# codelaboratoryltd/bng

Measured on NVIDIA H100. Metric: Mpps, higher is better.
Workload: dtype u8/u32/u64 integer

## Files before the change

### bng_b200/csrc/common.cuh

```cuda
#pragma once

#include <cuda_runtime.h>
#include <stdint.h>

typedef unsigned long long u64;
typedef uint32_t u32;
typedef uint16_t u16;
typedef uint8_t u8;

enum {
    ST_AS = 0,
    ST_AS_ALLOWED = 0, ST_AS_DROPPED, ST_AS_LOGGED, ST_AS_V4_VIOL, ST_AS_V6_VIOL, ST_AS_UNKNOWN_MAC,
    ST_QOS = 6,
    ST_QOS_PASS_PKTS = 6, ST_QOS_DROP_PKTS, ST_QOS_PASS_BYTES, ST_QOS_DROP_BYTES,
    ST_NAT = 10,
    ST_NAT_SNAT = 10, ST_NAT_DNAT, ST_NAT_HAIRPIN, ST_NAT_DROPPED, ST_NAT_PASSED, ST_NAT_CREATED,
    ST_NAT_EXPIRED, ST_NAT_EXHAUST, ST_NAT_EIM_HIT, ST_NAT_EIM_MISS, ST_NAT_ALG, ST_NAT_CT_LOOKUPS, ST_NAT_CT_HITS,
    ST_DHCP = 23,
    ST_DHCP_TOTAL = 23, ST_DHCP_HIT, ST_DHCP_MISS, ST_DHCP_ERROR, ST_DHCP_EXPIRED, ST_DHCP_O82_PRESENT,
    ST_DHCP_O82_ABSENT, ST_DHCP_BCAST, ST_DHCP_UCAST, ST_DHCP_VLAN,
    ST_LRU_OVERFLOW = 33,
    ST_EV_LOST_SPOOF = 34,
    ST_EV_LOST_NATLOG = 35,
    ST_TABLE_FULL = 36,
    ST_NAT_COOP = 37,
    ST_NAT_SEQ = 38,
    ST_LRU_EVICT = 39,
    ST_COUNT = 40,
};

#define K_EMPTY 0xFFFFFFFFFFFFFFFFull
#define K_TOMB 0xFFFFFFFFFFFFFFFEull
#define K_BUSY 0xFFFFFFFFFFFFFFFDull

struct Tbl {
    u8 *slots;
    u32 *count;
    u32 mask;
    u32 home_mask;
    u32 slot_bytes;
    u32 voff;
    u32 max_entries;
    u32 key_size;
    u32 value_size;
    u32 vlayout;
    u32 lru;
};
#define LRU_NONE 0u
#define LRU_TS 1u
#define LRU_ANY 2u
#define LRU_WINDOW 16u

#define VL_SESSION 1u
#define VL_QOS 2u
#define QOS_RATE_COPY 8u
enum {
    SES_NAT_IP = 16,
    SES_NAT_PORT = 20,
    SES_EPOCH = 22,
    SES_OUT_LO = 24,
    SES_LAST_SEEN = 32,
    SES_ORIG_IP = 40,
    SES_STATE = 44,
    SES_ORIG_PORT = 48,
    SES_IN_LO = 56,
    SES_OUT_HI = 64,
    SES_IN_HI = 72,
    SES_CREATED = 80,
    SES_DEST_IP = 88,
    SES_DEST_PORT = 92,
    SES_PAD_A = 96,
    SES_PAD_B = 100,
};
__host__ __device__ __forceinline__ u32 ses_abi_to_slot(u32 a) {
    if (a < 4) return SES_NAT_IP + a;
    if (a < 6) return SES_NAT_PORT + (a - 4);
    if (a < 8) return SES_ORIG_PORT + (a - 6);
    if (a < 12) return SES_ORIG_IP + (a - 8);
    if (a < 16) return SES_DEST_IP + (a - 12);
    if (a < 20) return SES_DEST_PORT + (a - 16);
    if (a < 24) return SES_PAD_A + (a - 20);
    if (a < 32) return SES_LAST_SEEN + (a - 24);
    if (a < 40) return SES_CREATED + (a - 32);
    if (a < 44) return SES_OUT_LO + (a - 40);
    if (a < 48) return SES_OUT_HI + (a - 44);
    if (a < 52) return SES_IN_LO + (a - 48);
    if (a < 56) return SES_IN_HI + (a - 52);
    if (a < 60) return SES_OUT_LO + 4 + (a - 56);
    if (a < 64) return SES_OUT_HI + 4 + (a - 60);
    if (a < 68) return SES_IN_LO + 4 + (a - 64);
    if (a < 72) return SES_IN_HI + 4 + (a - 68);
    if (a < 76) return SES_STATE + (a - 72);
    return SES_PAD_B + (a - 76);
}
__host__ __device__ __forceinline__ u32 ses_hi_of(u32 lo_off) { return lo_off == SES_OUT_LO ? (u32)SES_OUT_HI : (u32)SES_IN_HI; }
#ifdef __CUDACC__
__device__ __forceinline__ void ses_touch(u8 *ses, u64 now, u32 seen, u32 epoch, bool stamped = false) {
    if (stamped) {
        atomicMax((unsigned long long *)(ses + SES_LAST_SEEN), (unsigned long long)now);
    } else if (seen != epoch) {
        *(u64 *)(ses + SES_LAST_SEEN) = now;
        *(u16 *)(ses + SES_EPOCH) = (u16)epoch;
    }
}
static __device__ __noinline__ void ses_count_carry(u8 *ses, u32 lo_off, u32 c, u32 w) {
    u64 add = w ? (1ull << 32) : 0;
    if (c) {
        add += 1;
        u64 old = atomicAdd((unsigned long long *)(ses + lo_off), 0xFFFFFFFF00000000ull);
        if ((old >> 32) == 0) add -= 1ull << 32;
    }
    if (add) atomicAdd((unsigned long long *)(ses + ses_hi_of(lo_off)), add);
}
__device__ __forceinline__ void ses_count(u8 *ses, u32 lo_off, u32 len) {
    const u64 old = atomicAdd((unsigned long long *)(ses + lo_off), 1ull | ((u64)len << 32));
    const u32 c = (u32)old == 0xFFFFFFFFu;
    const u32 w = (u32)(((old >> 32) + len + c) >> 32);
    if (c | w) ses_count_carry(ses, lo_off, c, w);
}
#endif

#define DIR_NONE 0xFFFFFFFFu
#define DIR_QOS_UNLIMITED 0x80000000u
#define DIR_SLOT_MASK 0x7FFFFFFFu

struct LpmTbl {
    u32 *ents;
    u32 *count;
    u32 max_entries;
};

struct EvRing {
    u8 *buf;
    u32 *count;
    u32 cap;
    u32 rec_bytes;
    u32 lost_stat;
    u32 pad;
};

struct DevCtx {
    Tbl bindings;
    Tbl qos_eg;
    Tbl qos_in;
    Tbl sub_nat;
    Tbl sessions;
    Tbl reverse;
    Tbl eim;
    Tbl hairpin;
    Tbl alg;
    Tbl sub_pools;
    Tbl vlan_pools;
    Tbl cid_subs;
    Tbl ip_pools;
    Tbl cid_map;
    Tbl subdir;
    LpmTbl ranges_v4;
    LpmTbl priv_ranges;
    u8 *as_config;
    u8 *nat_config;
    u8 *server_config;
    u8 *nat_pool;
    u64 *stats;
    EvRing spoof_ev;
    EvRing natlog_ev;
    const struct SmallTabs *small;
    u32 batch_seq;
    u32 epoch;
};

#define HP_SLOTS 2048
#define HP_EMPTY 0xFFFFFFFFu
struct __align__(16) SmallTabs {
    u32 as_cfg;
    u32 nat_flags;
    u32 alg_n;
    u32 hp_n;
    u32 alg_key[64];
    u8 alg_type[64];
    u32 hp_hash[HP_SLOTS];
};
static_assert(sizeof(SmallTabs) % 16 == 0, "bulk copies move multiples of 16 bytes");

__host__ __device__ __forceinline__ u32 hp_index(u32 ip) { return (ip * 0x9E3779B1u) >> 21; }

struct DevBatch {
    u8 *pkts;
    const u32 *off16;
    u32 *len;
    u8 *verdict;
    u32 *priority;
    u32 n;
    u32 stride;
    u64 now;
    u32 base;
    u32 cap;
    u64 arena_len;
    const u64 *nowv;
    u32 kshift;
};
__device__ __forceinline__ void pdl_wait() { asm volatile("griddepcontrol.wait;" ::: "memory"); }
#define KEY_BITS 21
#define KEY_LEN_SAT 0x7FEu
__host__ __device__ __forceinline__ u32 key_mask_of(u32 kshift) { return kshift ? (1u << kshift) - 1 : 0xFFFFFFFFu; }
__device__ __forceinline__ u32 key_pack(u32 key, u32 len, u32 kshift) {
    return kshift ? key | ((len < KEY_LEN_SAT ? len : KEY_LEN_SAT) << kshift) : key;
}
#define FRAME_WIDE_OK(b, p) ((((uintptr_t)(p)) & 31) == 0 && (u64)((p) - (b).pkts) + 64 <= (b).arena_len)

__host__ __device__ __forceinline__ u64 mix64(u64 x) {
    x ^= x >> 33;
    x *= 0xff51afd7ed558ccdull;
    x ^= x >> 33;
    x *= 0xc4ceb9fe1a85ec53ull;
    x ^= x >> 33;
    return x;
}

__host__ __device__ __forceinline__ u64 splitmix64(u64 x) {
    x += 0x9e3779b97f4a7c15ull;
    x = (x ^ (x >> 30)) * 0xbf58476d1ce4e5b9ull;
    x = (x ^ (x >> 27)) * 0x94d049bb133111ebull;
    return x ^ (x >> 31);
}

__device__ __forceinline__ u16 bswap16(u16 x) { return (u16)((x << 8) | (x >> 8)); }
__device__ __forceinline__ u32 bswap32(u32 x) { return __byte_perm(x, 0, 0x0123); }

__device__ __forceinline__ u32 hash_word(u64 k, u32 seed) {
    u32 h = ((u32)k * 0x9E3779B1u) ^ ((u32)(k >> 32) * 0x85EBCA77u) ^ seed;
    h ^= h >> 16;
    h *= 0x7FEB352Du;
    h ^= h >> 15;
    return h;
}

template <int KW>
__device__ __forceinline__ u32 tbl_hash(const u64 *k) {
    u32 h = 0x2545F491u;
#pragma unroll
    for (int i = 0; i < KW; i++) h = hash_word(k[i], h);
    return h;
}

__device__ __forceinline__ u8 *tbl_slot(const Tbl &t, u32 i) { return t.slots + (size_t)i * t.slot_bytes; }

__device__ __forceinline__ u64 ld_vol64(const u8 *p) { return *(volatile const u64 *)p; }

template <int KW, bool VOL, bool SKIP_BUSY = false>
__device__ __forceinline__ u8 *tbl_find(const Tbl &t, const u64 *k) {
    if (k[0] >= K_BUSY) return nullptr;
    u32 i = (u32)tbl_hash<KW>(k) & t.home_mask;
    for (u32 probe = 0; probe <= t.mask; probe++) {
        u8 *s = tbl_slot(t, i);
        u64 w0 = VOL ? ld_vol64(s) : *(const u64 *)s;
        if (VOL && !SKIP_BUSY) {
            while (w0 == K_BUSY) {
                __nanosleep(32);
                w0 = ld_vol64(s);
            }
        }
        if (w0 == K_EMPTY) return nullptr;
        if (w0 == k[0]) {
            bool eq = true;
#pragma unroll
            for (int j = 1; j < KW; j++) eq = eq && (((const u64 *)s)[j] == k[j]);
            if (eq) return s;
        }
        i = (i + 1) & t.mask;
    }
    return nullptr;
}

__device__ __forceinline__ bool tbl_evict_near(const Tbl &t, u32 home, u64 *stats) {
    const u32 mode = t.lru & 0xff, ts_off = t.lru >> 8;
    for (u32 attempt = 0; attempt < 16; attempt++) {
        u8 *best = nullptr;
        u64 best_ts = ~0ull, best_w = 0;
        for (u32 j = 0; j < LRU_WINDOW; j++) {
            u8 *s = t.slots + (size_t)((home + (attempt >> 1) * LRU_WINDOW + j) & t.mask) * t.slot_bytes;
            const u64 w0 = *(volatile const u64 *)s;
            if (w0 >= K_BUSY) continue;
            const u64 ts = mode == LRU_TS ? *(volatile const u64 *)(s + ts_off) : j;
            if (ts < best_ts) {
                best_ts = ts;
                best = s;
                best_w = w0;
            }
        }
        if (best && atomicCAS((u64 *)best, best_w, K_TOMB) == best_w) {
            atomicSub(t.count, 1u);
            if (stats) atomicAdd(&stats[ST_LRU_EVICT], 1ull);
            return true;
        }
    }
    return false;
}

#define PROBE_W 2
template <int KW>
__device__ __forceinline__ u8 *tbl_find_ins(const Tbl &t, const u64 *k, u32 *ins) {
    *ins = 0xFFFFFFFFu;
    if (k[0] >= K_BUSY) return nullptr;
    u32 i = (u32)tbl_hash<KW>(k) & t.home_mask;
    for (u32 probe = 0; probe <= t.mask; probe += PROBE_W) {
        u64 w[PROBE_W];
#pragma unroll
        for (int j = 0; j < PROBE_W; j++) w[j] = ld_vol64(tbl_slot(t, (i + j) & t.mask));
#pragma unroll
        for (int j = 0; j < PROBE_W; j++) {
            const u32 si = (i + j) & t.mask;
            if (w[j] == K_EMPTY) {
                if (*ins == 0xFFFFFFFFu) *ins = si;
                return nullptr;
            }
            if (w[j] == K_TOMB && *ins == 0xFFFFFFFFu) *ins = si;
            if (w[j] == k[0]) {
                u8 *s = tbl_slot(t, si);
                bool eq = true;
#pragma unroll
                for (int q = 1; q < KW; q++) eq = eq && (((volatile const u64 *)s)[q] == k[q]);
                if (eq) return s;
            }
        }
        i = (i + PROBE_W) & t.mask;
    }
    return nullptr;
}
template <int KW>
__device__ __forceinline__ bool tbl_has(const Tbl &t, const u64 *k) {
    u32 ins;
    return tbl_find_ins<KW>(t, k, &ins) != nullptr;
}
template <int KW>
__device__ __forceinline__ u8 *tbl_claim_at(const Tbl &t, u32 ins, const u64 *k) {
    if (ins == 0xFFFFFFFFu) return nullptr;
    u8 *s = tbl_slot(t, ins);
    const u64 got = atomicCAS((u64 *)s, K_EMPTY, K_BUSY);
    if (got != K_EMPTY && !(got == K_TOMB && atomicCAS((u64 *)s, K_TOMB, K_BUSY) == K_TOMB)) return nullptr;
#pragma unroll
    for (int j = 1; j < KW; j++) ((u64 *)s)[j] = k[j];
    return s;
}
__device__ __forceinline__ void tbl_cas3(const Tbl &a, u32 ia, const Tbl &b, u32 ib, const Tbl &c, u32 ic, u64 got[3]) {
    got[0] = got[1] = got[2] = K_BUSY;
    if (ia != 0xFFFFFFFFu) got[0] = atomicCAS((u64 *)tbl_slot(a, ia), K_EMPTY, K_BUSY);
    if (ib != 0xFFFFFFFFu) got[1] = atomicCAS((u64 *)tbl_slot(b, ib), K_EMPTY, K_BUSY);
    if (ic != 0xFFFFFFFFu) got[2] = atomicCAS((u64 *)tbl_slot(c, ic), K_EMPTY, K_BUSY);
}
template <int KW>
__device__ __forceinline__ u8 *tbl_claim_finish(const Tbl &t, u32 ins, u64 got, const u64 *k) {
    if (ins == 0xFFFFFFFFu) return nullptr;
    u8 *s = tbl_slot(t, ins);
    if (got != K_EMPTY && !(got == K_TOMB && atomicCAS((u64 *)s, K_TOMB, K_BUSY) == K_TOMB)) return nullptr;
#pragma unroll
    for (int j = 1; j < KW; j++) ((u64 *)s)[j] = k[j];
    return s;
}

__device__ __forceinline__ bool tbl_reserve(const Tbl &t, u32 n) {
    if (atomicAdd(t.count, n) + n > t.max_entries) {
        atomicSub(t.count, n);
        return false;
    }
    return true;
}
__device__ __forceinline__ void tbl_unreserve(const Tbl &t, u32 n) {
    if (n) atomicSub(t.count, n);
}

template <int KW>
__device__ __forceinline__ const u8 *tbl_find_conv(const Tbl &t, const u64 *k) {
    const unsigned m = __activemask();
    const u8 *res = nullptr;
    bool done = k[0] >= K_BUSY;
    u32 i = (u32)tbl_hash<KW>(k) & t.home_mask, left = t.mask + 1;
    while (__any_sync(m, !done)) {
        if (!done) {
            const u8 *s = tbl_slot(t, i);
            const u64 w0 = *(const u64 *)s;
            if (w0 == K_EMPTY) {
                done = true;
            } else {
                bool eq = w0 == k[0];
#pragma unroll
                for (int j = 1; j < KW; j++) eq = eq && (((const u64 *)s)[j] == k[j]);
                if (eq) {
                    res = s;
                    done = true;
                } else {
                    i = (i + 1) & t.mask;
                    done = --left == 0;
                }
            }
        }
    }
    return res;
}

template <int KW, bool SKIP_BUSY = false, bool RESERVED = false>
__device__ __forceinline__ u8 *tbl_find_or_claim(const Tbl &t, const u64 *k, bool *created, u32 *pending = nullptr,
                                                 u64 *stats = nullptr) {
    *created = false;
    if (k[0] >= K_BUSY) return nullptr;
    const u32 home = (u32)tbl_hash<KW>(k) & t.home_mask;
    u32 i = home;
    int tomb = -1;
    for (u32 probe = 0; probe <= t.mask + 1;) {
        const bool wrapped = probe == t.mask + 1;
        if (wrapped && tomb < 0) return nullptr;
        u8 *s = tbl_slot(t, i);
        u64 w0 = wrapped ? K_EMPTY : ld_vol64(s);
        while (!SKIP_BUSY && w0 == K_BUSY) {
            __nanosleep(32);
            w0 = ld_vol64(s);
        }
        if (w0 == k[0]) {
            bool eq = true;
#pragma unroll
            for (int j = 1; j < KW; j++) eq = eq && (((volatile const u64 *)s)[j] == k[j]);
            if (eq) return s;
        }
        if (w0 == K_TOMB && tomb < 0) tomb = (int)i;
        if (w0 == K_EMPTY) {
            u32 target = tomb >= 0 ? (u32)tomb : i;
            u64 expect = tomb >= 0 ? K_TOMB : K_EMPTY;
            u8 *ts = tbl_slot(t, target);
            if (RESERVED) {
            } else if (pending) {
                if (*(volatile u32 *)t.count + *pending >= t.max_entries && !(t.lru && tbl_evict_near(t, home, stats))) return nullptr;
            } else if (atomicAdd(t.count, 1u) >= t.max_entries) {
                if (!(t.lru && tbl_evict_near(t, home, stats))) {
                    atomicSub(t.count, 1u);
                    return nullptr;
                }
            }
            u64 old = atomicCAS((u64 *)ts, expect, K_BUSY);
            if (old == expect) {
#pragma unroll
                for (int j = 1; j < KW; j++) ((u64 *)ts)[j] = k[j];
                *created = true;
                if (pending) ++*pending;
                return ts;
            }
            if (!pending && !RESERVED) atomicSub(t.count, 1u);
            if (tomb >= 0 || wrapped) {
                tomb = -1;
                i = home;
                probe = 0;
            }
            continue;
        }
        i = (i + 1) & t.mask;
        probe++;
    }
    return nullptr;
}

template <bool FENCE = true>
__device__ __forceinline__ void tbl_publish(u8 *slot, u64 k0) {
    if (FENCE) __threadfence();
    *(volatile u64 *)slot = k0;
}

template <int KW>
__device__ __forceinline__ bool tbl_erase(const Tbl &t, const u64 *k) {
    u8 *s = tbl_find<KW, true>(t, k);
    if (!s) return false;
    u64 old = atomicCAS((u64 *)s, k[0], K_TOMB);
    if (old != k[0]) return false;
    atomicSub(t.count, 1u);
    return true;
}

__device__ __forceinline__ bool lpm_match(const LpmTbl &t, u32 addr, u32 maxlen) {
    u32 n = *t.count;
    u32 a = bswap32(addr);
    for (u32 i = 0; i < n; i++) {
        u32 pl = t.ents[3 * i];
        if (pl > maxlen) continue;
        u32 e = bswap32(t.ents[3 * i + 1]);
        u32 m = pl == 0 ? 0u : (0xFFFFFFFFu << (32 - pl));
        if (((a ^ e) & m) == 0) return true;
    }
    return false;
}

struct BlockStats {
    u64 v[ST_COUNT];
};

__device__ __forceinline__ void bstats_init(BlockStats &s) {
    for (int i = threadIdx.x; i < ST_COUNT; i += blockDim.x) s.v[i] = 0;
    __syncthreads();
}
__device__ __forceinline__ void bstats_add(BlockStats &s, int idx, u64 v) { atomicAdd(&s.v[idx], v); }
__device__ __forceinline__ void bstats_flush(BlockStats &s, u64 *g) {
    __syncthreads();
    for (int i = threadIdx.x; i < ST_COUNT; i += blockDim.x)
        if (s.v[i]) atomicAdd(&g[i], s.v[i]);
}

__device__ __forceinline__ void warp_stat_flush(BlockStats &s, int idx, u32 v) {
    u32 t = __reduce_add_sync(0xffffffffu, v);
    if ((threadIdx.x & 31) == 0 && t) atomicAdd(&s.v[idx], (u64)t);
}
__device__ __forceinline__ void warp_stat_flush64(BlockStats &s, int idx, u64 v) {
#pragma unroll
    for (int o = 16; o > 0; o >>= 1) v += __shfl_xor_sync(0xffffffffu, v, o);
    if ((threadIdx.x & 31) == 0 && v) atomicAdd(&s.v[idx], v);
}

__device__ __forceinline__ void bstats_inc_pred(BlockStats &s, int idx, bool pred) {
    unsigned m = __ballot_sync(__activemask(), pred);
    if (pred) {
        int leader = __ffs(m) - 1;
        if ((threadIdx.x & 31) == leader) atomicAdd(&s.v[idx], (u64)__popc(m));
    }
}

__device__ __forceinline__ u8 *ev_reserve(const DevCtx &c, const EvRing &r, u32 frame_idx) {
    u32 pos = atomicAdd(r.count, 1u);
    if (pos >= r.cap) {
        atomicSub(r.count, 1u);
        atomicAdd(&c.stats[r.lost_stat], 1ull);
        return nullptr;
    }
    u8 *rec = r.buf + (size_t)pos * r.rec_bytes;
    *(uint2 *)(rec + r.rec_bytes - 8) = make_uint2(frame_idx, c.batch_seq);
    return rec;
}

__device__ __forceinline__ u64 frame_now(const DevBatch &b, u32 i) { return b.nowv ? b.nowv[i] : b.now; }
__device__ __forceinline__ u32 frame_dlen(const DevBatch &b, u32 len) { return (b.cap && len > b.cap) ? b.cap : len; }
__device__ __forceinline__ u8 *frame_ptr(const DevBatch &b, u32 i) {
    return b.pkts + (b.off16 ? (size_t)b.off16[i] * 16 : (size_t)i * b.stride);
}
__device__ __forceinline__ u16 rd16(const u8 *p, u32 off) { return *(const u16 *)(p + off); }
__device__ __forceinline__ u32 rd32(const u8 *p, u32 off) {
    return (u32)rd16(p, off) | ((u32)rd16(p, off + 2) << 16);
}
__device__ __forceinline__ void wr16(u8 *p, u32 off, u16 v) { *(u16 *)(p + off) = v; }
__device__ __forceinline__ void wr32(u8 *p, u32 off, u32 v) {
    wr16(p, off, (u16)v);
    wr16(p, off + 2, (u16)(v >> 16));
}

struct Hdr64 {
    u32 w[16];
    __device__ __forceinline__ u8 b8(u32 off) const { return (u8)(w[off >> 2] >> ((off & 3) * 8)); }
    __device__ __forceinline__ u16 b16(u32 off) const {
        return (u16)(w[off >> 2] >> ((off & 2) * 8));
    }
    __device__ __forceinline__ u32 b32(u32 off) const {
        return (off & 2) ? (u32)(w[off >> 2] >> 16) | (w[(off >> 2) + 1] << 16) : w[off >> 2];
    }
    __device__ __forceinline__ void s16(u32 off, u16 v) {
        u32 sh = (off & 2) * 8;
        w[off >> 2] = (w[off >> 2] & ~(0xFFFFu << sh)) | ((u32)v << sh);
    }
    __device__ __forceinline__ void s32(u32 off, u32 v) {
        s16(off, (u16)v);
        s16(off + 2, (u16)(v >> 16));
    }
};

__device__ __forceinline__ void hdr_load(Hdr64 &h, const u8 *p, u32 len) {
#pragma unroll
    for (int c = 0; c < 4; c++) {
        uint4 v = make_uint4(0, 0, 0, 0);
        if ((u32)c * 16 < len) v = *(const uint4 *)(p + c * 16);
        h.w[4 * c + 0] = v.x;
        h.w[4 * c + 1] = v.y;
        h.w[4 * c + 2] = v.z;
        h.w[4 * c + 3] = v.w;
    }
}
__device__ __forceinline__ void hdr_store_chunk(const Hdr64 &h, u8 *p, int c) {
    *(uint4 *)(p + c * 16) = make_uint4(h.w[4 * c], h.w[4 * c + 1], h.w[4 * c + 2], h.w[4 * c + 3]);
}

struct __align__(16) U256 {
    u32 w[8];
};
#define BNG_LDG128(r, q)                                                                                         \
    asm volatile("ld.global.v4.u32 {%0,%1,%2,%3}, [%4];"                                                         \
                 : "=r"((r)[0]), "=r"((r)[1]), "=r"((r)[2]), "=r"((r)[3])                                        \
                 : "l"(q)                                                                                        \
                 : "memory")
#define BNG_STG128(q, w)                                                                                         \
    asm volatile("st.global.v4.u32 [%0], {%1,%2,%3,%4};" ::"l"(q), "r"((w)[0]), "r"((w)[1]), "r"((w)[2]),         \
                 "r"((w)[3])                                                                                     \
                 : "memory")
__device__ __forceinline__ U256 ldg256(const void *p) {
    U256 r;
    const u8 *q = (const u8 *)p;
    BNG_LDG128(&r.w[0], q);
    BNG_LDG128(&r.w[4], q + 16);
    return r;
}
__device__ __forceinline__ void stg256(void *p, const u32 *w) {
    u8 *q = (u8 *)p;
    BNG_STG128(q, &w[0]);
    BNG_STG128(q + 16, &w[4]);
}
#undef BNG_LDG128
#undef BNG_STG128
__device__ __forceinline__ void hdr_load_wide(Hdr64 &h, const u8 *p, u32 len, bool wide) {
    if (wide) {
        U256 a, b;
#pragma unroll
        for (int k = 0; k < 8; k++) a.w[k] = b.w[k] = 0;
        if (len > 0) a = ldg256(p);
        if (len > 32) b = ldg256(p + 32);
#pragma unroll
        for (int k = 0; k < 8; k++) {
            h.w[k] = a.w[k];
            h.w[8 + k] = b.w[k];
        }
    } else {
        hdr_load(h, p, len);
    }
}

__device__ __forceinline__ u64 mac_key(const Hdr64 &h, u32 off) {
    if (off == 6)
        return ((u64)__byte_perm(h.w[1], 0, 0x4423) << 32) | __byte_perm(h.w[2], 0, 0x0123);
    u64 k = 0;
#pragma unroll
    for (int i = 0; i < 6; i++) k = (k << 8) | h.b8(off + i);
    return k;
}

__device__ __forceinline__ u16 csum_fold32(u32 c) {
    c = (c & 0xffff) + (c >> 16);
    c = (c & 0xffff) + (c >> 16);
    return (u16)~c;
}
__device__ __forceinline__ u16 csum_upd32(u16 csum, u32 old_val, u32 new_val) {
    u32 sum = ~((u32)csum) & 0xffff;
    sum += ~old_val & 0xffff;
    sum += ~(old_val >> 16) & 0xffff;
    sum += new_val & 0xffff;
    sum += new_val >> 16;
    return csum_fold32(sum);
}
__device__ __forceinline__ u16 csum_upd16(u16 csum, u16 old_val, u16 new_val) {
    u32 sum = ~((u32)csum) & 0xffff;
    sum += ~(u32)old_val & 0xffff;
    sum += (u32)new_val & 0xffff;
    return csum_fold32(sum);
}

__device__ __forceinline__ void smem_stage_begin(void *smem_dst, const void *gsrc, u32 bytes, u64 *bar) {
    if (threadIdx.x == 0) {
        u32 bar_a = (u32)__cvta_generic_to_shared(bar);
        u32 dst_a = (u32)__cvta_generic_to_shared(smem_dst);
        asm volatile("mbarrier.init.shared::cta.b64 [%0], 1;" ::"r"(bar_a));
        asm volatile("fence.mbarrier_init.release.cluster;" ::: "memory");
        asm volatile("mbarrier.arrive.expect_tx.shared::cta.b64 _, [%0], %1;" ::"r"(bar_a), "r"(bytes) : "memory");
        asm volatile("cp.async.bulk.shared::cluster.global.mbarrier::complete_tx::bytes [%0], [%1], %2, [%3];" ::"r"(dst_a),
                     "l"(gsrc), "r"(bytes), "r"(bar_a)
                     : "memory");
    }
    __syncthreads();
}
__device__ __forceinline__ void smem_stage_wait(u64 *bar) {
    u32 bar_a = (u32)__cvta_generic_to_shared(bar);
    u32 done = 0;
    while (!done) {
        asm volatile(
            "{\n\t.reg .pred p;\n\t"
            "mbarrier.try_wait.parity.shared::cta.b64 p, [%1], 0;\n\t"
            "selp.u32 %0, 1, 0, p;\n\t}"
            : "=r"(done)
            : "r"(bar_a)
            : "memory");
    }
}

__device__ __forceinline__ bool hp_contains(const SmallTabs &st, u32 ip) {
    if (ip == HP_EMPTY) return (st.hp_n >> 31) != 0;
    if ((st.hp_n & 0x7fffffffu) == 0) return false;
    u32 i = hp_index(ip);
    for (u32 probe = 0; probe < HP_SLOTS; probe++) {
        u32 v = st.hp_hash[i];
        if (v == ip) return true;
        if (v == HP_EMPTY) return false;
        i = (i + 1) & (HP_SLOTS - 1);
    }
    return false;
}
__device__ __forceinline__ int alg_find(const SmallTabs &st, u32 key) {
    for (u32 i = 0; i < st.alg_n; i++)
        if (st.alg_key[i] == key) return (int)i;
    return -1;
}

template <int KW>
__device__ __forceinline__ u8 *tbl_finish(const Tbl &t, const u64 *k, u32 i0, u64 w0, bool rest_eq) {
    if (k[0] >= K_BUSY) return nullptr;
    if (w0 == k[0] && rest_eq) return tbl_slot(t, i0);
    if (w0 == K_EMPTY) return nullptr;
    u32 i = (i0 + 1) & t.mask;
    for (u32 probe = 1; probe <= t.mask; probe++) {
        u8 *s = tbl_slot(t, i);
        u64 w = *(const u64 *)s;
        if (w == K_EMPTY) return nullptr;
        if (w == k[0]) {
            bool eq = true;
#pragma unroll
            for (int j = 1; j < KW; j++) eq = eq && (((const u64 *)s)[j] == k[j]);
            if (eq) return s;
        }
        i = (i + 1) & t.mask;
    }
    return nullptr;
}
```

### bng_b200/csrc/pipe_classify.cuh

```cuda
#pragma once

#define CLASSIFY_BLOCKS 3
#define CLASSIFY_BLOCKS_NAT 4
#define CLASSIFY_BPS(AS) ((AS) ? CLASSIFY_BLOCKS : CLASSIFY_BLOCKS_NAT)

template <bool AS, bool QOS, bool TC = false, bool ACCT = false>
__global__ void __launch_bounds__(BLOCK, CLASSIFY_BPS(AS))
    k_pipe_classify(const __grid_constant__ DevCtx c, const __grid_constant__ DevBatch b, u32 *skey, u32 *sval, u32 *cnt, u32 *T,
                    u32 *attr) {
    __shared__ SmallTabs st;
    scratch_reset(cnt, T);
    __shared__ BlockStats bs;
    __shared__ u64 bar;
    smem_stage_begin(&st, c.small, (u32)sizeof(SmallTabs), &bar);
    bstats_init(bs);
    smem_stage_wait(&bar);
    const u32 lane = threadIdx.x & 31;
#define as_cfg (st.as_cfg)
#define nflags (st.nat_flags)
#define epoch (c.epoch)
    AsCnt cn = {0, 0};
    u32 n_snat = 0, n_qpass = 0, n_qbytes = 0;
    for (u32 base = blockIdx.x * BLOCK + (threadIdx.x & ~31u); base < b.n; base += gridDim.x * BLOCK) {
        const u32 i = base + lane;
        const bool act = i < b.n;
        const u32 len = act ? b.len[i] : 0;
        const u32 dlen = frame_dlen(b, len);
        u8 *p = act ? frame_ptr(b, i) : b.pkts;
        const bool wide = __all_sync(0xffffffffu, !act || FRAME_WIDE_OK(b, p));
        Hdr64 h;
        hdr_load_wide(h, p, dlen, wide);

        const bool ip4 = dlen >= 34 && h.b16(12) == ETH_P_IP_LE;
        const u32 saddr = h.b32(26), daddr = h.b32(30), proto = h.b8(23);
        const bool ihl5 = (h.b8(14) & 0x0f) == 5;
        u64 mk = mac_key(h, 6);
        const u32 bi = tbl_hash<1>(&mk) & c.bindings.home_mask;
        u64 sk = saddr;
        const u32 di = tbl_hash<1>(&sk) & c.subdir.home_mask;
        u16 sport, dport;
        if (proto == 1) {
            sport = h.b16(38);
            dport = 0;
        } else {
            sport = h.b16(34);
            dport = h.b16(36);
        }
        u64 key[2];
        key[0] = (u64)saddr | ((u64)daddr << 32);
        key[1] = (u64)sport | ((u64)dport << 16) | ((u64)proto << 32);
        const u32 hi = tbl_hash<2>(key) & c.sessions.mask;
        BindVal bv;
        U256 s0;
        bv.s.w[0] = bv.s.w[1] = s0.w[0] = s0.w[1] = 0xFFFFFFFFu;
        s0.w[2] = s0.w[3] = 0;
        uint4 d0 = make_uint4(0xFFFFFFFFu, 0xFFFFFFFFu, 0xFFFFFFFFu, 0xFFFFFFFFu);
        const u8 *bslot0 = tbl_slot(c.bindings, bi);
        u8 *sslot0 = tbl_slot(c.sessions, hi);
        if (AS && dlen >= 14) bv.s = ldg256(bslot0);
        if (ip4) {
            d0 = *(const uint4 *)tbl_slot(c.subdir, di);
            s0 = ldg256(sslot0);
        }
        const u64 kw0 = (u64)s0.w[0] | ((u64)s0.w[1] << 32), kw1 = (u64)s0.w[2] | ((u64)s0.w[3] << 32);

        int v = TC_OK;
        if (AS) {
            const u8 *bind = nullptr;
            if (dlen >= 14 && mk < K_BUSY) {
                const u64 w0 = (u64)bv.s.w[0] | ((u64)bv.s.w[1] << 32);
                if (w0 == mk) {
                    bind = bslot0;
                } else if (w0 != K_EMPTY) {
                    bind = tbl_finish<1>(c.bindings, &mk, bi, w0, true);
                    if (bind) bv.s = ldg256(bind);
                }
            }
            __syncwarp();
            bv.has = bind != nullptr;
            v = antispoof_eval(c, nullptr, h, dlen, i + b.base, act ? frame_now(b, i) : 0, bv, as_cfg, cn);
            __syncwarp();
        }
        const bool alive = act && v != TC_SHOT && ip4;

        u32 nat_slot = DIR_NONE, qos_slot = DIR_NONE, dir_idx = ACCT ? DIR_NONE : 0;
        if (alive) {
            const u64 k0 = (u64)d0.x | ((u64)d0.y << 32);
            if (k0 == sk) {
                nat_slot = d0.z, qos_slot = d0.w, dir_idx = di;
            } else if (k0 != K_EMPTY) {
                const u8 *de = tbl_finish<1>(c.subdir, &sk, di, k0, true);
                if (de) {
                    const u64 w = *(const u64 *)(de + 8);
                    nat_slot = (u32)w;
                    qos_slot = (u32)(w >> 32);
                    dir_idx = (u32)((de - c.subdir.slots) >> 4);
                }
            }
        }
        __syncwarp();
        if (!QOS) qos_slot = DIR_NONE;
        const bool defer = TC && alive && qos_slot != DIR_NONE && !(qos_slot & DIR_QOS_UNLIMITED);
        const bool priv = alive && !defer && is_private_ip(saddr);
        const bool has_sub = priv && nat_slot != DIR_NONE;
        if (priv && !has_sub) bstats_add(bs, ST_NAT_PASSED, 1);
        bool go = has_sub && ihl5 && (proto == 6 ? dlen >= 54u : ((proto == 17 || proto == 1) && dlen >= 42u));
        if (go && proto != 1 && (nflags & (proto == 6 ? (NATF_ALG_FTP | NATF_ALG_SIP) : NATF_ALG_SIP)) && st.alg_n) {
            int ax = alg_find(st, ((u32)bswap16(dport) << 16) | proto);
            if (ax >= 0) {
                bstats_add(bs, ST_NAT_ALG, 1);
                const u8 *sub = tbl_slot(c.sub_nat, nat_slot);
                nat_log(c, i + b.base, frame_now(b, i), 7, *(const u32 *)(sub + 32), saddr, 0, sport, 0, daddr, dport, (u8)proto, st.alg_type[ax]);
                go = false;
            }
        }
        __syncwarp();
        if (go && (nflags & NATF_HAIRPIN) && hp_contains(st, daddr)) bstats_add(bs, ST_NAT_HAIRPIN, 1);
        __syncwarp();
        u8 *ses = go ? tbl_finish<2>(c.sessions, key, hi, kw0, kw1 == key[1]) : nullptr;
        __syncwarp();

        bool miss = go && !ses;
        if (ses) {
            uint2 tr = make_uint2(s0.w[4], s0.w[5]);
            if (ses != sslot0) tr = *(const uint2 *)(ses + SES_NAT_IP);
            const u32 nat_ip = tr.x;
            const u16 nat_port = (u16)tr.y;
            ses_touch(ses, frame_now(b, i), tr.y >> 16, epoch, b.nowv != nullptr);
            ses_count(ses, SES_OUT_LO, len);
            h.s32(26, nat_ip);
            h.s16(24, csum_upd32(h.b16(24), saddr, nat_ip));
            if (proto == 6) {
                h.s16(34, nat_port);
                u16 ck = csum_upd32(h.b16(50), saddr, nat_ip);
                h.s16(50, csum_upd16(ck, sport, nat_port));
            } else if (proto == 17) {
                h.s16(34, nat_port);
                u16 ck = h.b16(40);
                if (ck != 0) {
                    ck = csum_upd32(ck, saddr, nat_ip);
                    ck = csum_upd16(ck, sport, nat_port);
                    if (ck == 0) ck = 0xffff;
                    h.s16(40, ck);
                }
            } else {
                h.s16(38, nat_port);
                h.s16(36, csum_upd16(h.b16(36), sport, nat_port));
            }
            if (wide) {
                stg256(p, &h.w[0]);
                if (proto == 6 || dlen >= 64)
                    stg256(p + 32, &h.w[8]);
                else
                    hdr_store_chunk(h, p, 2);
            } else {
                hdr_store_chunk(h, p, 1);
                hdr_store_chunk(h, p, 2);
                if (proto == 6) hdr_store_chunk(h, p, 3);
            }
            n_snat++;
        }
        __syncwarp();

        if (has_sub && !ihl5) {
            NatOut o = nat_egress_one<false>(c, bs, p, tbl_slot(c.sub_nat, nat_slot), len, dlen, i + b.base, frame_now(b, i), nullptr, true, b.nowv != nullptr);
            v = o.verdict;
            miss = o.miss;
        }
        __syncwarp();

        u32 okey = NO_KEY, oval = i;
        if (alive && v != TC_SHOT) {
            if (qos_slot != DIR_NONE && (qos_slot & DIR_QOS_UNLIMITED) && !miss) {
                n_qpass++;
                n_qbytes += len;
            } else if (qos_slot != DIR_NONE || miss) {
                okey = key_pack(dir_idx, len, b.kshift);
            }
            if (miss) oval |= MISS_FLAG;
            if (defer) oval |= DEFER_FLAG;
        }
        if (act) {
            b.verdict[i] = (u8)v;
            skey[i] = okey;
            sval[i] = oval;
        }
        if (ACCT) {
            u32 aw = alive ? dir_idx : DIR_NONE;
            if (act && !ip4 && dlen >= 30 && h.b16(12) == ETH_P_IP_LE && (!AS || v != TC_SHOT)) {
                const u8 *de = tbl_find<1, false>(c.subdir, &sk);
                if (de) aw = (u32)((de - c.subdir.slots) >> 4);
            }
            if (act) attr[i] = aw;
        }
        if (AS) ascnt_spill(bs, cn);
        if (QOS && __any_sync(0xffffffffu, n_qbytes >= 0x04000000u)) {
            warp_stat_flush(bs, ST_QOS_PASS_BYTES, n_qbytes);
            n_qbytes = 0;
        }
    }
#undef as_cfg
#undef nflags
#undef epoch
    if (AS) ascnt_flush(bs, cn);
    warp_stat_flush(bs, ST_NAT_SNAT, n_snat);
    if (QOS) {
        warp_stat_flush(bs, ST_QOS_PASS_PKTS, n_qpass);
        warp_stat_flush(bs, ST_QOS_PASS_BYTES, n_qbytes);
    }
    bstats_flush(bs, c.stats);
}
```

Baseline: 4211.

## Load and store packet headers cooperatively across warp via shared-memory transpose

Replaces per-thread wide header loads and stores with a warp-cooperative scheme. Four lanes each fetch one 16-byte chunk of a frame, the chunks are transposed through a per-warp shared-memory slice, and each lane then reads its own 64-byte header; NAT rewrites go back through the same path. The goal is better coalescing of global accesses to packet data. In exchange it adds shuffles, shared-memory traffic (about 2.5KB per warp), extra syncwarps and possible occupancy pressure.

```diff
diff --git a/bng_b200/csrc/common.cuh b/bng_b200/csrc/common.cuh
--- a/bng_b200/csrc/common.cuh
+++ b/bng_b200/csrc/common.cuh
@@ -623,6 +623,51 @@
     }
 }
 
+struct WarpSlice {
+    uint4 f[32][5];
+};
+
+__device__ __forceinline__ void hdr_load_coop(Hdr64 &h, WarpSlice &s, const u8 *p, u32 len, bool wide, u32 lane) {
+    const u32 c = lane & 3;
+    uint4 v[4];
+#pragma unroll
+    for (int q = 0; q < 4; q++) {
+        const u32 f = 8 * q + (lane >> 2);
+        const u8 *fp = (const u8 *)__shfl_sync(0xffffffffu, (unsigned long long)p, f);
+        const u32 fl = __shfl_sync(0xffffffffu, len, f);
+        v[q] = make_uint4(0, 0, 0, 0);
+        if (wide ? fl > (c < 2 ? 0u : 32u) : c * 16 < fl) v[q] = *(const uint4 *)(fp + c * 16);
+    }
+#pragma unroll
+    for (int q = 0; q < 4; q++) s.f[8 * q + (lane >> 2)][c] = v[q];
+    __syncwarp();
+#pragma unroll
+    for (int k = 0; k < 4; k++) {
+        const uint4 x = s.f[lane][k];
+        h.w[4 * k + 0] = x.x;
+        h.w[4 * k + 1] = x.y;
+        h.w[4 * k + 2] = x.z;
+        h.w[4 * k + 3] = x.w;
+    }
+    __syncwarp();
+}
+
+__device__ __forceinline__ void hdr_store_coop(const Hdr64 &h, WarpSlice &s, u8 *p, u32 mask, u32 lane) {
+    if (mask)
+#pragma unroll
+        for (int k = 0; k < 4; k++) s.f[lane][k] = make_uint4(h.w[4 * k], h.w[4 * k + 1], h.w[4 * k + 2], h.w[4 * k + 3]);
+    __syncwarp();
+    const u32 c = lane & 3;
+#pragma unroll
+    for (int q = 0; q < 4; q++) {
+        const u32 f = 8 * q + (lane >> 2);
+        u8 *fp = (u8 *)__shfl_sync(0xffffffffu, (unsigned long long)p, f);
+        const u32 fm = __shfl_sync(0xffffffffu, mask, f);
+        if ((fm >> c) & 1) *(uint4 *)(fp + c * 16) = s.f[f][c];
+    }
+    __syncwarp();
+}
+
 __device__ __forceinline__ u64 mac_key(const Hdr64 &h, u32 off) {
     if (off == 6)
         return ((u64)__byte_perm(h.w[1], 0, 0x4423) << 32) | __byte_perm(h.w[2], 0, 0x0123);
diff --git a/bng_b200/csrc/pipe_classify.cuh b/bng_b200/csrc/pipe_classify.cuh
--- a/bng_b200/csrc/pipe_classify.cuh
+++ b/bng_b200/csrc/pipe_classify.cuh
@@ -12,10 +12,12 @@
     scratch_reset(cnt, T);
     __shared__ BlockStats bs;
     __shared__ u64 bar;
+    __shared__ WarpSlice slices[BLOCK / 32];
     smem_stage_begin(&st, c.small, (u32)sizeof(SmallTabs), &bar);
     bstats_init(bs);
     smem_stage_wait(&bar);
     const u32 lane = threadIdx.x & 31;
+    WarpSlice &sl = slices[threadIdx.x >> 5];
 #define as_cfg (st.as_cfg)
 #define nflags (st.nat_flags)
 #define epoch (c.epoch)
@@ -29,7 +31,7 @@
         u8 *p = act ? frame_ptr(b, i) : b.pkts;
         const bool wide = __all_sync(0xffffffffu, !act || FRAME_WIDE_OK(b, p));
         Hdr64 h;
-        hdr_load_wide(h, p, dlen, wide);
+        hdr_load_coop(h, sl, p, dlen, wide, lane);
 
         const bool ip4 = dlen >= 34 && h.b16(12) == ETH_P_IP_LE;
         const u32 saddr = h.b32(26), daddr = h.b32(30), proto = h.b8(23);
@@ -121,6 +123,7 @@
         __syncwarp();
 
         bool miss = go && !ses;
+        u32 smask = 0;
         if (ses) {
             uint2 tr = make_uint2(s0.w[4], s0.w[5]);
             if (ses != sslot0) tr = *(const uint2 *)(ses + SES_NAT_IP);
@@ -147,20 +150,14 @@
                 h.s16(38, nat_port);
                 h.s16(36, csum_upd16(h.b16(36), sport, nat_port));
             }
-            if (wide) {
-                stg256(p, &h.w[0]);
-                if (proto == 6 || dlen >= 64)
-                    stg256(p + 32, &h.w[8]);
-                else
-                    hdr_store_chunk(h, p, 2);
-            } else {
-                hdr_store_chunk(h, p, 1);
-                hdr_store_chunk(h, p, 2);
-                if (proto == 6) hdr_store_chunk(h, p, 3);
-            }
+            if (wide)
+                smask = (proto == 6 || dlen >= 64) ? 0xfu : 0x7u;
+            else
+                smask = proto == 6 ? 0xeu : 0x6u;
             n_snat++;
         }
         __syncwarp();
+        if (__any_sync(0xffffffffu, smask)) hdr_store_coop(h, sl, p, smask, lane);
 
         if (has_sub && !ihl5) {
             NatOut o = nat_egress_one<false>(c, bs, p, tbl_slot(c.sub_nat, nat_slot), len, dlen, i + b.base, frame_now(b, i), nullptr, true, b.nowv != nullptr);
```

Result: no change. 4287, median of 6 (+1.8%).
